# bcsefercik/markerless-robot-camera-calibration

Hardware: AMD Instinct MI355X
Metric: point-cloud frames/sec at 200k pts/frame (higher is better)
Workload: dtype f32

## Files before the change

markerless-robot-camera-calibration_amd/csrc/sv_conv.hip:

```cpp
#include <stdarg.h>
#include <stdio.h>
#include <stdlib.h>
#include <vector>

#include "sv_conv_params.h"

namespace sv {

static thread_local char g_last_instance[128] = "";
static thread_local double g_want_scale_override = -1.0;
static thread_local double g_tail_override = -1.0;
void note_instance(const char* fmt, ...) {
  va_list ap;
  va_start(ap, fmt);
  vsnprintf(g_last_instance, sizeof(g_last_instance), fmt, ap);
  va_end(ap);
}
#ifndef SV_CONV_WANT_SCALE_DEFAULT
#define SV_CONV_WANT_SCALE_DEFAULT 0.3
#endif
#ifndef SV_CONV_TAIL_DEFAULT
#define SV_CONV_TAIL_DEFAULT 0.15
#endif
constexpr int chunk_for(int tm, int waves_n) {
  if (waves_n == 1) return tm <= 64 ? 128 : 64;
  if (waves_n == 2) return tm <= 32 ? 128 : (tm <= 64 ? 64 : 32);
  return tm <= 16 ? 128 : (tm <= 32 ? 64 : 32);
}

constexpr int fused_offsets(int cpo) { return cpo == 0 ? 1 : (cpo < 8 ? 27 : (128 / cpo > 0 ? 128 / cpo : 1)); }
constexpr int lds_row_stride(int kc) {
  for (int sa = kc + 2;; ++sa)
    if (sa % 64 == 34 || (sa % 4 == 0 && (sa / 4) % 2 == 1)) return sa;
}

template <int TM_, int WAVES_N, int NT, int CPO = 0>
struct ConvCfg {
  static constexpr int WAVES_M = 4 / WAVES_N;
  static constexpr int MR = TM_ / WAVES_M / 16;
  static constexpr int TN = WAVES_N * NT * 16;
  static constexpr int GK = fused_offsets(CPO);
  static constexpr int KC = CPO ? (GK * CPO + 3) / 4 * 4 : chunk_for(TM_, WAVES_N);
  static constexpr int SA = lds_row_stride(KC);
  static constexpr int PFD_RAW = MR * NT >= 6 ? 1 : (8 + MR * NT - 1) / (MR * NT);
  static constexpr int PFD = PFD_RAW > KC / 4 ? KC / 4 : PFD_RAW;
  static constexpr bool USE_FULL = (MR * NT == 1) || (TM_ == 32 && WAVES_N == 4 && NT == 3) || (TM_ == 16 && NT == 3);
  static constexpr int F4_PER_ROW = KC / 4;
  static constexpr int ROWS_PER_PASS = 256 / F4_PER_ROW;
  static constexpr int A_F4 = (TM_ + ROWS_PER_PASS - 1) / ROWS_PER_PASS;
  static_assert(MR >= 1, "tile too small for the wave layout");
  static constexpr size_t lds_bytes(int K) { return (size_t)(2 * TM_ * SA + K * TM_) * sizeof(float); }
};

template <int TM_, int WAVES_N, int NT, bool FAST, int CPO = 0, bool RING = false, bool FULL = false>
__device__ __forceinline__ void conv_tile_body(const ConvParams& p, const int bidx, const int tile_base) {
  static_assert(FAST || !FULL, "FULL is a refinement of the FAST form");
  using Cfg = ConvCfg<TM_, WAVES_N, NT, CPO>;
  constexpr int MR = Cfg::MR, TN = Cfg::TN, A_F4 = Cfg::A_F4, KC = Cfg::KC, SA = Cfg::SA, GK = Cfg::GK;
  constexpr int PFD = RING ? Cfg::PFD : 1;
  constexpr int ROWS_PER_PASS = Cfg::ROWS_PER_PASS;
  constexpr int SUBS = TM_ / 16;
  extern __shared__ __attribute__((aligned(16))) float lds[];
  float* As = lds;
  int* idx_s = (int*)(lds + 2 * TM_ * SA);

  const int tid = threadIdx.x;
  const int lane = tid & 63;
  const int wid = __builtin_amdgcn_readfirstlane(tid >> 6);
  const int wm = wid / WAVES_N, wn = wid % WAVES_N;
  unsigned long long trace_t0 = 0, trace_t_loop = 0, trace_t_epi = 0;
  int trace_steps = 0;
  if (p.trace) trace_t0 = wall_clock64();
  const int ny = (p.Cout + TN - 1) / TN;
  constexpr int SUB_PER_PLAN_TILE = PLAN_TILE / TM_;
  const int t_lin = bidx / ny;
  const int t128 = tile_base + t_lin / SUB_PER_PLAN_TILE;
  const int p128 = p.tile_order ? p.tile_order[t128] : ((int)(p.Vpad / PLAN_TILE) - 1 - t128);
  const int tile = p128 * SUB_PER_PLAN_TILE + (t_lin % SUB_PER_PLAN_TILE);
  const int n0 = (bidx % ny) * TN;
  const int64_t row0 = (int64_t)tile * TM_;
  const int li = lane & 15, lq = lane >> 4;
  const int K = p.K, Cin = p.Cin, Cout = p.Cout;
  const int col0 = n0 + wn * NT * 16 + NT * li;
  const bool cols_full = col0 + NT <= Cout;

  f32x4 acc[MR][NT];
#pragma unroll
  for (int s = 0; s < MR; ++s)
#pragma unroll
    for (int n = 0; n < NT; ++n) acc[s][n] = (f32x4){0.f, 0.f, 0.f, 0.f};

  if (p.acc_init) {
    if constexpr (FAST) {
      const __amdgpu_buffer_rsrc_t rsrc_acc = __builtin_amdgcn_make_buffer_rsrc((void*)p.acc_init, 0, (int)p.acc_bytes, 0x00020000);
      int o_acc[MR][4];
      load_perm_rows<MR>(p, row0 + wm * MR * 16, lane >> 4, o_acc);
#pragma unroll
      for (int s = 0; s < MR; ++s)
#pragma unroll
        for (int reg = 0; reg < 4; ++reg) {
          const auto v = buffer_load_floats<NT>(
              rsrc_acc, o_acc[s][reg] >= 0 ? (uint32_t)o_acc[s][reg] * (uint32_t)(p.acc_ld * 4) + (uint32_t)col0 * 4u : BUF_ABSENT, 0u);
#pragma unroll
          for (int n = 0; n < NT; ++n) acc[s][n][reg] = v[n];
        }
    } else {
#pragma unroll
      for (int s = 0; s < MR; ++s)
#pragma unroll
        for (int reg = 0; reg < 4; ++reg) {
          const int64_t r = row0 + wm * MR * 16 + s * 16 + (lane >> 4) * 4 + reg;
          const int64_t o = p.perm ? (int64_t)p.perm[r] : (r < p.V_out ? r : -1);
#pragma unroll
          for (int n = 0; n < NT; ++n) acc[s][n][reg] = (o >= 0 && col0 + n < Cout) ? p.acc_init[o * p.acc_ld + col0 + n] : 0.0f;
        }
    }
  }
  uint32_t dense_mask = (1u << SUBS) - 1u;
  if (p.submask == nullptr) {
    const int64_t rem = p.V_out - row0;
    const int nsub = rem >= TM_ ? SUBS : (int)((rem + 15) / 16);
    dense_mask = (1u << nsub) - 1u;
  }
  if constexpr (FAST) {
    constexpr int STAGE_IT = (32 * TM_ + 255) / 256;
    int n_st[STAGE_IT];
#pragma unroll
    for (int it = 0; it < STAGE_IT; ++it) {
      const int e = tid + 256 * it;
      const int k = e / TM_, r = e % TM_;
      n_st[it] = -1;
      if (e < K * TM_) {
        if (p.nbr_s)
          n_st[it] = p.nbr_s[(int64_t)k * p.Vpad + row0 + r];
        else
          n_st[it] = (row0 + r < p.V_out) ? (int)(row0 + r) : -1;
      }
    }
#pragma unroll
    for (int it = 0; it < STAGE_IT; ++it) {
      const int e = tid + 256 * it;
      if (e < K * TM_) idx_s[e] = (int)(n_st[it] >= 0 ? (uint32_t)n_st[it] * (uint32_t)(p.in_ld * 4) : BUF_ABSENT);
    }
  } else {
    for (int e = tid; e < K * TM_; e += 256) {
      const int k = e / TM_, r = e - k * TM_;
      int n;
      if (p.nbr_s)
        n = p.nbr_s[(int64_t)k * p.Vpad + row0 + r];
      else
        n = (row0 + r < p.V_out) ? (int)(row0 + r) : -1;
      idx_s[e] = n;
    }
  }
  const __amdgpu_buffer_rsrc_t rsrc_in = __builtin_amdgcn_make_buffer_rsrc((void*)p.in, 0, (int)p.in_bytes, 0x00020000);
  const __amdgpu_buffer_rsrc_t rsrc_w = __builtin_amdgcn_make_buffer_rsrc((void*)p.W, 0, (int)p.w_bytes, 0x00020000);

  const int64_t sm_word = row0 / PLAN_TILE;
  const int sm_shift = (int)((row0 % PLAN_TILE) / 16);
  uint32_t my_sm = 0;
  if (lane < K) my_sm = p.submask ? ((p.submask[sm_word * K + lane] >> sm_shift) & ((1u << SUBS) - 1u)) : dense_mask;
  const uint32_t amask = (uint32_t)__ballot(my_sm != 0);
  auto fused_mask = [&](int k0) -> uint32_t {
    uint32_t m = 0;
#pragma unroll
    for (int g = 0; g < GK; ++g) m |= (uint32_t)__builtin_amdgcn_readlane((int)my_sm, min(k0 + g, 31));
    return m;
  };
  int k_n, c_n = 0;
  uint32_t sm_n = 0;
  bool have_n;
  if (CPO) {
    k_n = 0;
    while (k_n < K && (sm_n = fused_mask(k_n)) == 0) k_n += GK;
    have_n = k_n < K;
  } else {
    k_n = amask ? __builtin_ctz(amask) : K;
    sm_n = amask ? (uint32_t)__builtin_amdgcn_readlane((int)my_sm, k_n) : 0u;
    have_n = amask != 0;
  }
  auto advance = [&]() {
    if (CPO) {
      k_n += GK;
      while (k_n < K && (sm_n = fused_mask(k_n)) == 0) k_n += GK;
      have_n = k_n < K;
      return;
    }
    c_n += KC;
    if (c_n >= Cin) {
      c_n = 0;
      const uint32_t rest = amask & ~((2u << k_n) - 1u);
      have_n = rest != 0;
      k_n = have_n ? __builtin_ctz(rest) : K;
      sm_n = (uint32_t)__builtin_amdgcn_readlane((int)my_sm, have_n ? k_n : 0);
    }
  };

  float4 ra[A_F4];
  const int a_cc = (tid % Cfg::F4_PER_ROW) * 4;
  const int a_r = tid / Cfg::F4_PER_ROW;

  const uint32_t col_bytes = (uint32_t)a_cc * 4u;
  const int cin_rem = Cin % KC;
  const uint32_t col_last = (cin_rem == 0 || a_cc < cin_rem) ? col_bytes : 0u - (uint32_t)(Cin - cin_rem) * 4u;
  auto load_a = [&](int k, int c0, uint32_t sm) {
#pragma unroll
    for (int j = 0; j < A_F4; ++j) {
      const int r = a_r + ROWS_PER_PASS * j;
      if (FAST) {
        const int rr = (A_F4 * ROWS_PER_PASS > TM_) ? min(r, TM_ - 1) : r;
        if (CPO) {
          const int kk = k + a_cc / (CPO ? CPO : 1);
          uint32_t off = (uint32_t)idx_s[min(kk, K - 1) * TM_ + rr];
          if (kk >= K) off = BUF_ABSENT;
          const f32x4 v = buffer_load_floats<4>(rsrc_in, off + (uint32_t)(a_cc % (CPO ? CPO : 1)) * 4u, 0u);
          ra[j] = make_float4(v[0], v[1], v[2], v[3]);
        } else {
          const uint32_t off = (uint32_t)idx_s[k * TM_ + rr];
          const uint32_t cb = (!FULL && c0 + KC > Cin) ? col_last : col_bytes;
          const f32x4 v = buffer_load_floats<4>(rsrc_in, off + cb, (uint32_t)c0 * 4u);
          ra[j] = make_float4(v[0], v[1], v[2], v[3]);
        }
        (void)sm;
      } else if (CPO) {
        float e[4] = {0.f, 0.f, 0.f, 0.f};
        if (r < TM_ && ((sm >> (r >> 4)) & 1u)) {
#pragma unroll
          for (int q = 0; q < 4; ++q) {
            const int i = a_cc + q, kk = k + i / (CPO ? CPO : 1), c = i % (CPO ? CPO : 1);
            if (i < GK * CPO && kk < K) {
              const int n = idx_s[kk * TM_ + r];
              if (n >= 0) e[q] = p.in[(int64_t)n * p.in_ld + c];
            }
          }
        }
        ra[j] = make_float4(e[0], e[1], e[2], e[3]);
      } else {
        float4 v = make_float4(0.f, 0.f, 0.f, 0.f);
        if (r < TM_ && ((sm >> (r >> 4)) & 1u)) {
          const int n = idx_s[k * TM_ + r];
          const int c = c0 + a_cc;
          if (n >= 0) {
            const float* src = p.in + (int64_t)n * p.in_ld + c;
            if (p.vec_a) {
              if (c < Cin) v = *(const float4*)src;
            } else {
              if (c + 0 < Cin) v.x = src[0];
              if (c + 1 < Cin) v.y = src[1];
              if (c + 2 < Cin) v.z = src[2];
              if (c + 3 < Cin) v.w = src[3];
            }
          }
        }
        ra[j] = v;
      }
    }
  };
  auto store_a = [&](float* dstbuf, uint32_t sm) {
#pragma unroll
    for (int j = 0; j < A_F4; ++j) {
      const int r = a_r + ROWS_PER_PASS * j;
      if (r < TM_ && (FAST || ((sm >> (r >> 4)) & 1u))) {
        float2* dst = (float2*)(dstbuf + r * SA + a_cc);
        dst[0] = make_float2(ra[j].x, ra[j].y);
        dst[1] = make_float2(ra[j].z, ra[j].w);
      }
    }
  };

  typedef float bvec_t __attribute__((ext_vector_type(NT)));
  typedef float bvec_load_t __attribute__((ext_vector_type(NT), aligned(4)));
  bvec_t b[KC / 4];
  const int b_off = lq * Cout + col0;
  const uint32_t b_off_bytes = (uint32_t)b_off * 4u;
  auto step_weights = [&](int k, int c0) -> const float* { return p.W + ((int64_t)k * Cin + c0) * Cout; };
  auto cols_of = [&](int k, int c0) { return CPO ? min(GK, K - k) * CPO : min(KC, Cin - c0); };
  auto ksteps_of = [&](int k, int c0) { return (cols_of(k, c0) + 3) >> 2; };
  auto load_b = [&](const float* wstep, int k, int c0, int ksteps_valid, int ks, bvec_t& dst) {
    if (FAST) {
      const uint32_t row = (uint32_t)(k * Cin + c0 + (ks < ksteps_valid ? 4 * ks : 0));
      dst = buffer_load_floats<NT>(rsrc_w, b_off_bytes, row * (uint32_t)Cout * 4u);
      (void)wstep;
    } else {
      const int i = 4 * ks + lq;
      const float* src = p.W + ((int64_t)k * Cin + c0 + i) * Cout + col0;
      const bool row_ok = i < cols_of(k, c0);
#pragma unroll
      for (int n = 0; n < NT; ++n) dst[n] = (row_ok && col0 + n < Cout) ? src[n] : 0.0f;
    }
  };

  __syncthreads();
  if (have_n) {
    int k_c = k_n, c_c = c_n;
    uint32_t sm_c = sm_n;
    load_a(k_c, c_c, sm_c);
#pragma unroll
    for (int ks = 0; ks < KC / 4; ++ks) load_b(step_weights(k_c, c_c), k_c, c_c, ksteps_of(k_c, c_c), ks, b[ks]);
    store_a(As, sm_c);
    advance();
    int k_x = k_n, c_x = c_n;
    uint32_t sm_x = sm_n;
    bool have_x = have_n;
    __syncthreads();
    int buf = 0;
    if (p.trace) trace_t_loop = wall_clock64();

    auto step = [&]() -> bool {
      if (FAST || have_x) load_a(have_x ? k_x : 0, have_x ? c_x : 0, have_x ? sm_x : 0u);
      const float* a_base = As + buf * (TM_ * SA) + (wm * MR * 16 + li) * SA + lq;
      const uint32_t smw = (sm_c >> (wm * MR)) & ((1u << MR) - 1u);
      const int ksteps = ksteps_of(k_c, c_c);
      const int kb = have_x ? k_x : 0;
      const int cb = have_x ? c_x : 0;
      const float* wnext = step_weights(kb, cb);
      const int ksteps_next = ksteps_of(kb, cb);
      {
        auto reload_b = [&](int ks) {
          if (FULL) {
            b[ks] = buffer_load_floats<NT>(rsrc_w, b_off_bytes, (uint32_t)(kb * Cin + cb + 4 * ks) * (uint32_t)Cout * 4u);
          } else if (FAST || have_x) {
            load_b(wnext, kb, cb, ksteps_next, ks, b[ks]);
          }
        };
        auto mfma_row = [&](int ks, const float (&a)[MR]) {
#pragma unroll
          for (int s = 0; s < MR; ++s) {
            if ((MR == 1 && Cfg::WAVES_M == 1) || ((smw >> s) & 1u)) {
#pragma unroll
              for (int n = 0; n < NT; ++n)
                acc[s][n] = __builtin_amdgcn_mfma_f32_16x16x4f32(a[s], b[ks][n], acc[s][n], 0, 0, 0);
            }
          }
        };
        if constexpr (PFD == 1) {
          float a_cur[MR];
#pragma unroll
          for (int s = 0; s < MR; ++s) a_cur[s] = a_base[s * 16 * SA];
#pragma unroll
          for (int ks = 0; ks < KC / 4; ++ks) {
            if (FULL || ks < ksteps) {
              float a_nx[MR];
              if (ks + 1 < KC / 4) {
#pragma unroll
                for (int s = 0; s < MR; ++s) a_nx[s] = a_base[s * 16 * SA + (ks + 1) * 4];
                if (FULL) __builtin_amdgcn_sched_barrier(0);
              }
              mfma_row(ks, a_cur);
              if (ks + 1 < KC / 4) {
#pragma unroll
                for (int s = 0; s < MR; ++s) a_cur[s] = a_nx[s];
              }
            }
            reload_b(ks);
            if (FULL) __builtin_amdgcn_sched_barrier(0);
          }
        } else {
          float a_ring[PFD + 1][MR];
#pragma unroll
          for (int d = 0; d < PFD; ++d)
#pragma unroll
            for (int s = 0; s < MR; ++s) a_ring[d][s] = a_base[s * 16 * SA + d * 4];
#pragma unroll
          for (int ks = 0; ks < KC / 4; ++ks) {
            if (FULL || ks < ksteps) {
              if (ks + PFD < KC / 4) {
#pragma unroll
                for (int s = 0; s < MR; ++s)
                  a_ring[(ks + PFD) % (PFD + 1)][s] = a_base[s * 16 * SA + (ks + PFD) * 4];
                if (FULL) __builtin_amdgcn_sched_barrier(0);
              }
              mfma_row(ks, a_ring[ks % (PFD + 1)]);
            }
            reload_b(ks);
            if (FULL) __builtin_amdgcn_sched_barrier(0);
          }
        }
      }
      ++trace_steps;
      if (!have_x) return false;
      store_a(As + (buf ^ 1) * (TM_ * SA), sm_x);
      k_c = k_x;
      c_c = c_x;
      sm_c = sm_x;
      advance();
      k_x = k_n;
      c_x = c_n;
      sm_x = sm_n;
      have_x = have_n;
      __syncthreads();
      buf ^= 1;
      return true;
    };
    while (step()) {
    }
  }

  if (p.trace) trace_t_epi = wall_clock64();
  float sc[NT], sh[NT];
#pragma unroll
  for (int n = 0; n < NT; ++n) {
    const bool ok = col0 + n < Cout;
    sc[n] = (p.scale && ok) ? p.scale[col0 + n] : 1.0f;
    sh[n] = (p.shift && ok) ? p.shift[col0 + n] : 0.0f;
  }
  if constexpr (FAST) {
    epilogue_buffered<MR, NT>(p, acc, row0 + wm * MR * 16, lq, col0);
  } else
#pragma unroll
  for (int s = 0; s < MR; ++s) {
#pragma unroll
    for (int reg = 0; reg < 4; ++reg) {
      const int64_t r = row0 + wm * MR * 16 + s * 16 + lq * 4 + reg;
      int64_t o;
      if (p.perm)
        o = p.perm[r];
      else
        o = (r < p.V_out) ? r : -1;
      if (o < 0) continue;
      float y[NT];
#pragma unroll
      for (int n = 0; n < NT; ++n) {
        float v = acc[s][n][reg];
        if (p.scale)
          v = __builtin_fmaf(v, sc[n], sh[n]);
        else if (p.shift)
          v = v + sh[n];
        y[n] = v;
      }
      if (p.residual) {
        const float* res = p.residual + o * p.res_ld + col0;
#pragma unroll
        for (int n = 0; n < NT; ++n)
          if (col0 + n < Cout) y[n] = y[n] + res[n];
      }
      float* dst = p.out + o * p.out_ld + col0;
#pragma unroll
      for (int n = 0; n < NT; ++n) {
        float v = y[n];
        if (p.act == SV_ACT_RELU)
          v = v < 0.f ? 0.f : v;
        else if (p.act == SV_ACT_LEAKY_RELU)
          v = v > 0.f ? v : v * p.slope;
        if (col0 + n < Cout) dst[n] = v;
      }
    }
  }
  if (p.trace && tid == 0) {
    unsigned long long* t = p.trace + (size_t)blockIdx.x * 4;
    t[0] = trace_t0;
    t[1] = wall_clock64();
    t[2] = ((unsigned long long)__builtin_amdgcn_s_getreg((31 << 11) | 20) << 32) |
           (unsigned)__builtin_amdgcn_s_getreg((31 << 11) | 4);
    const unsigned long long pro = trace_t_loop ? ((trace_t_loop - trace_t0) >> 4) & 0xffffull : 0ull;
    const unsigned long long epi = ((t[1] - trace_t_epi) >> 4) & 0xffffull;
    t[3] = (unsigned long long)(unsigned)trace_steps | (pro << 32) | (epi << 48);
  }
}

template <int TM_, int WAVES_N, int NT, bool FAST, int CPO = 0, bool RING = false, bool FULL = false>
__global__ __launch_bounds__(256) void conv_fwd_kernel(ConvParams p) {
  conv_tile_body<TM_, WAVES_N, NT, FAST, CPO, RING, FULL>(p, (int)blockIdx.x, 0);
}

template <int TM_, int TAIL_TM, int WAVES_N, int NT, bool FAST>
__global__ __launch_bounds__(256) void conv_fwd_dual_kernel(ConvParams p) {
  if ((int)blockIdx.x < p.main_blocks)
    conv_tile_body<TM_, WAVES_N, NT, FAST>(p, (int)blockIdx.x, 0);
  else
    conv_tile_body<TAIL_TM, WAVES_N, NT, FAST>(p, (int)blockIdx.x - p.main_blocks, p.main_tiles128);
}

template <class Launch>
static int launch_traced(ConvParams& q, unsigned grid, int tm, int wn, int nt, hipStream_t stream, Launch&& launch) {
  static const char* trace_path = getenv("SV_CONV_TRACE");
  q.trace = nullptr;
  if (trace_path) SV_HIP(hipMalloc((void**)&q.trace, (size_t)grid * 4 * sizeof(unsigned long long)));
  launch();
  SV_LAUNCH_CHECK();
  if (q.trace) {
    std::vector<unsigned long long> host((size_t)grid * 4);
    SV_HIP(hipStreamSynchronize(stream));
    SV_HIP(hipMemcpy(host.data(), q.trace, host.size() * sizeof(unsigned long long), hipMemcpyDeviceToHost));
    SV_HIP(hipFree(q.trace));
    if (FILE* f = fopen(trace_path, "ab")) {
      const long long hdr[8] = {0x5356545243ll, (long long)grid, tm, wn, nt, q.ny, q.K, q.Cin};
      fwrite(hdr, sizeof(hdr), 1, f);
      fwrite(host.data(), sizeof(unsigned long long), host.size(), f);
      fclose(f);
    }
  }
  return SV_OK;
}

template <int TM_, int WAVES_N, int NT, int CPO = 0>
static int launch_conv(const ConvParams& p, hipStream_t stream) {
  using Cfg = ConvCfg<TM_, WAVES_N, NT, CPO>;
  ConvParams q = p;
  q.ntiles = (int)(p.Vpad / TM_);
  q.ny = (p.Cout + Cfg::TN - 1) / Cfg::TN;
  dim3 grid((unsigned)(q.ntiles * q.ny));
  const bool fast = p.vec_a && p.buf_ok && (p.Cout % Cfg::TN == 0);
  const bool ring = Cfg::PFD > 1 && grid.x <= 1024;
  constexpr bool F = (CPO % 4 == 0);
  const size_t lds = Cfg::lds_bytes(p.K);
  const bool full = Cfg::USE_FULL && (CPO ? (p.K % Cfg::GK == 0) : (p.Cin % Cfg::KC == 0));
  const int rc = launch_traced(q, grid.x, TM_, WAVES_N, NT, stream, [&] {
    if (F && fast && full) {
      if (ring)
        hipLaunchKernelGGL((conv_fwd_kernel<TM_, WAVES_N, NT, F, CPO, (Cfg::PFD > 1), (F && Cfg::USE_FULL)>), grid, dim3(256), lds, stream, q);
      else
        hipLaunchKernelGGL((conv_fwd_kernel<TM_, WAVES_N, NT, F, CPO, false, (F && Cfg::USE_FULL)>), grid, dim3(256), lds, stream, q);
    } else if (F && fast) {
      if (ring)
        hipLaunchKernelGGL((conv_fwd_kernel<TM_, WAVES_N, NT, F, CPO, (Cfg::PFD > 1)>), grid, dim3(256), lds, stream, q);
      else
        hipLaunchKernelGGL((conv_fwd_kernel<TM_, WAVES_N, NT, F, CPO, false>), grid, dim3(256), lds, stream, q);
    } else {
      if (ring)
        hipLaunchKernelGGL((conv_fwd_kernel<TM_, WAVES_N, NT, false, CPO, (Cfg::PFD > 1)>), grid, dim3(256), lds, stream, q);
      else
        hipLaunchKernelGGL((conv_fwd_kernel<TM_, WAVES_N, NT, false, CPO, false>), grid, dim3(256), lds, stream, q);
    }
  });
  if (rc != SV_OK) return rc;
  {
    const bool f = F && fast;
    if (CPO)
      note_instance("conv_fwd_kernel<%d, %d, %d, fused %d>|fast=%d,ring=%d,full=%d", TM_, WAVES_N, NT, CPO, (int)f, (int)ring,
                    (int)(f && full));
    else
      note_instance("conv_fwd_kernel<%d, %d, %d>|fast=%d,ring=%d,full=%d", TM_, WAVES_N, NT, (int)f, (int)ring, (int)(f && full));
  }
  return SV_OK;
}

template <int TM_, int TAIL_TM, int WAVES_N, int NT>
static int launch_conv_dual(const ConvParams& p, hipStream_t stream, double tail_fraction) {
  using Main = ConvCfg<TM_, WAVES_N, NT, 0>;
  using Tail = ConvCfg<TAIL_TM, WAVES_N, NT, 0>;
  const bool fast = p.vec_a && p.buf_ok && (p.Cout % Main::TN == 0);
  const int n128 = (int)(p.Vpad / PLAN_TILE);
  const int tail128 = (int)(n128 * tail_fraction);
  if (!fast || !p.tile_order || tail128 < 1 || tail128 >= n128) return SV_ERR_INVALID;
  ConvParams q = p;
  q.ny = p.Cout / Main::TN;
  q.main_tiles128 = n128 - tail128;
  q.main_blocks = q.main_tiles128 * (PLAN_TILE / TM_) * q.ny;
  q.ntiles = (int)(p.Vpad / TM_);
  const unsigned grid = (unsigned)(q.main_blocks + tail128 * (PLAN_TILE / TAIL_TM) * q.ny);
  const size_t lds = Main::lds_bytes(p.K) > Tail::lds_bytes(p.K) ? Main::lds_bytes(p.K) : Tail::lds_bytes(p.K);
  const int rc = launch_traced(q, grid, TM_, WAVES_N, NT, stream, [&] {
    hipLaunchKernelGGL((conv_fwd_dual_kernel<TM_, TAIL_TM, WAVES_N, NT, true>), dim3(grid), dim3(256), lds, stream, q);
  });
  if (rc != SV_OK) return rc;
  note_instance("conv_fwd_dual_kernel<%d, %d, %d, %d>|fast=1,ring=0,full=0", TM_, TAIL_TM, WAVES_N, NT);
  return SV_OK;
}

struct Candidate {
  int tm, wn, nt;
  int64_t want;
  int cpo;
};

template <int TM_, int WAVES_N, int NT, int CPO = 0>
static bool try_launch(const Candidate& c, const ConvParams& p, hipStream_t stream, int& rc) {
  if (c.tm == TM_ && c.wn == WAVES_N && c.nt == NT && c.cpo == CPO) {
    rc = launch_conv<TM_, WAVES_N, NT, CPO>(p, stream);
    return true;
  }
  return false;
}

static int launch_candidate(const Candidate& c, const ConvParams& p, hipStream_t stream) {
  int rc = SV_ERR_INVALID;
  if (try_launch<128, 4, 3>(c, p, stream, rc) || try_launch<128, 2, 3>(c, p, stream, rc) ||
      try_launch<128, 1, 3>(c, p, stream, rc) || try_launch<64, 4, 3>(c, p, stream, rc) ||
      try_launch<64, 2, 3>(c, p, stream, rc) || try_launch<64, 1, 3>(c, p, stream, rc) ||
      try_launch<32, 4, 3>(c, p, stream, rc) || try_launch<32, 2, 3>(c, p, stream, rc) ||
      try_launch<16, 4, 3>(c, p, stream, rc) ||
      try_launch<128, 4, 2>(c, p, stream, rc) || try_launch<128, 2, 2>(c, p, stream, rc) ||
      try_launch<128, 1, 2>(c, p, stream, rc) || try_launch<64, 4, 2>(c, p, stream, rc) ||
      try_launch<64, 2, 2>(c, p, stream, rc) || try_launch<64, 1, 2>(c, p, stream, rc) ||
      try_launch<32, 4, 2>(c, p, stream, rc) || try_launch<32, 2, 2>(c, p, stream, rc) ||
      try_launch<16, 4, 2>(c, p, stream, rc) ||
      try_launch<64, 4, 1>(c, p, stream, rc) || try_launch<32, 4, 1>(c, p, stream, rc) ||
      try_launch<16, 4, 1>(c, p, stream, rc) || try_launch<128, 2, 1>(c, p, stream, rc) ||
      try_launch<64, 2, 1>(c, p, stream, rc) || try_launch<32, 2, 1>(c, p, stream, rc) ||
      try_launch<128, 1, 1>(c, p, stream, rc) || try_launch<64, 1, 1>(c, p, stream, rc) ||
      try_launch<64, 2, 1, 3>(c, p, stream, rc) || try_launch<32, 2, 1, 3>(c, p, stream, rc) ||
      try_launch<64, 2, 1, 32>(c, p, stream, rc) || try_launch<32, 2, 1, 32>(c, p, stream, rc) ||
      try_launch<32, 4, 1, 32>(c, p, stream, rc) || try_launch<16, 4, 1, 32>(c, p, stream, rc) ||
      try_launch<32, 4, 1, 64>(c, p, stream, rc) || try_launch<16, 4, 1, 64>(c, p, stream, rc))
    return rc;
  set_error("sv_conv_fwd: no kernel instance <%d,%d,%d> cpo %d", c.tm, c.wn, c.nt, c.cpo);
  return SV_ERR_INVALID;
}

static int64_t candidate_wgs(const Candidate& c, const ConvParams& p) {
  const int tn = c.wn * c.nt * 16;
  return (p.Vpad / c.tm) * ((p.Cout + tn - 1) / tn);
}

static int select_and_launch(const ConvParams& p, hipStream_t stream) {
  static const Candidate wide3[] = {{64, 4, 3, 2500}, {32, 4, 3, 1500}, {32, 2, 3, 0}};
  static const Candidate wide3_128[] = {{64, 4, 3, 2500}, {64, 4, 2, 1200}, {32, 4, 3, 1200}, {16, 4, 3, 0}};
  static const Candidate wide3_128_full[] = {{64, 4, 3, 2500}, {32, 4, 3, 1200}, {16, 4, 3, 0}};
  static const Candidate wide2[] = {{128, 4, 2, 1300}, {64, 4, 2, 1500}, {32, 4, 2, 1500}, {32, 2, 2, 0}};
  static const Candidate wide2_64[] = {{128, 4, 2, 1300}, {64, 4, 2, 1500}, {32, 4, 2, 1500}, {16, 4, 1, 0}};
  static const Candidate c64[] = {{64, 4, 1, 1500}, {32, 4, 1, 1500}, {16, 4, 1, 0}};
  static const Candidate c32[] = {{128, 2, 1, 1500}, {64, 2, 1, 1500}, {32, 2, 1, 0}};
  static const Candidate c16[] = {{128, 1, 1, 600}, {64, 1, 1, 0}};
  const Candidate* list;
  int n;
  const int Cout = p.Cout;
  if (Cout > 128 && (Cout % 192 == 0 || Cout % 96 == 0 || Cout > 2048)) {
    if (Cout % 128 != 0) { list = wide3; n = 3; }
    else if (p.Cin % 128 == 0 && p.vec_a) { list = wide3_128_full; n = 3; }
    else { list = wide3_128; n = 4; }
  }
  else if (Cout > 64) { list = Cout % 64 == 0 ? wide2_64 : wide2; n = 4; }
  else if (Cout > 32) { list = c64; n = 3; }
  else if (Cout > 16) { list = c32; n = 3; }
  else { list = c16; n = 2; }
  static const Candidate f3[] = {{64, 2, 1, 3000, 3}, {32, 2, 1, 0, 3}};
  static const Candidate f32_32[] = {{64, 2, 1, 3000, 32}, {32, 2, 1, 0, 32}};
  static const Candidate f32_64[] = {{32, 4, 1, 1500, 32}, {16, 4, 1, 0, 32}};
  static const Candidate f64_64[] = {{32, 4, 1, 1500, 64}, {16, 4, 1, 0, 64}};
  if (p.K > 1) {
    if (p.Cin == 3 && Cout > 16 && Cout <= 32) { list = f3; n = 2; }
    else if (p.Cin == 32 && p.vec_a && Cout == 32) { list = f32_32; n = 2; }
    else if (p.Cin == 32 && p.vec_a && Cout == 64) { list = f32_64; n = 2; }
    else if (p.Cin == 64 && p.vec_a && (Cout == 64 || Cout == 128)) { list = f64_64; n = 2; }
  }
  if (const char* f = getenv("SV_CONV_FORCE_RANGE")) {
    long long vmin = 0, vmax = 0;
    int cout = 0;
    Candidate c = {0, 0, 0, 0, 0};
    if (sscanf(f, "%lld:%lld:%d:%d,%d,%d", &vmin, &vmax, &cout, &c.tm, &c.wn, &c.nt) == 6 && p.Vpad >= vmin && p.Vpad <= vmax &&
        p.Cout == cout && p.K > 1)
      return launch_candidate(c, p, stream);
  }
  if (const char* f = getenv("SV_CONV_FORCE_DENSE")) {
    long long vmin = 0;
    int cout = 0;
    Candidate c = {0, 0, 0, 0, 0};
    if (sscanf(f, "%lld:%d:%d,%d,%d", &vmin, &cout, &c.tm, &c.wn, &c.nt) == 5 && p.Vpad >= vmin && p.Cout == cout && p.K == 1)
      return launch_candidate(c, p, stream);
  }
  if (const char* f = getenv("SV_CONV_FORCE")) {
    Candidate c = {0, 0, 0, 0, 0};
    if (sscanf(f, "%d,%d,%d,%d", &c.tm, &c.wn, &c.nt, &c.cpo) >= 3) return launch_candidate(c, p, stream);
  }
  static const double want_scale =
      getenv("SV_CONV_WANT_SCALE") ? atof(getenv("SV_CONV_WANT_SCALE")) : SV_CONV_WANT_SCALE_DEFAULT;
  static const double tail_fraction = getenv("SV_CONV_TAIL") ? atof(getenv("SV_CONV_TAIL")) : SV_CONV_TAIL_DEFAULT;
  const double ws = g_want_scale_override >= 0.0 ? g_want_scale_override : want_scale;
  const double tf = g_tail_override >= 0.0 ? g_tail_override : tail_fraction;
  for (int i = 0; i < n; ++i)
    if ((double)candidate_wgs(list[i], p) >= ws * (double)list[i].want) {
      const Candidate& c = list[i];
      if (c.tm == 64 && c.wn == 4 && c.nt == 3 && c.cpo == 0 && tf > 0.0 &&
          launch_conv_dual<64, 32, 4, 3>(p, stream, tf) == SV_OK)
        return SV_OK;
      return launch_candidate(c, p, stream);
    }
  return launch_candidate(list[n - 1], p, stream);
}

}

using namespace sv;

extern "C" const char* sv_conv_last_instance(void) { return sv::g_last_instance; }

extern "C" int sv_conv_set_dispatch(double want_scale, double tail_fraction) {
  SV_CHECK_ARG(tail_fraction < 1.0, "tail_fraction must be below 1");
  sv::g_want_scale_override = want_scale;
  sv::g_tail_override = tail_fraction;
  return SV_OK;
}

extern "C" int sv_conv_fwd(const float* in, int64_t V_in, int64_t in_ld, int Cin, const float* W, int K, int Cout,
                           const int32_t* perm, const int32_t* nbr_s, const uint32_t* submask,
                           const int32_t* tile_order, int64_t V_out, int64_t Vpad, const float* scale, const float* shift, const float* residual, int64_t res_ld,
                           int act, float slope, float* out, int64_t out_ld, sv_stream_t stream_) {
  return sv_conv_fwd_acc(in, V_in, in_ld, Cin, W, K, Cout, perm, nbr_s, submask, tile_order, V_out, Vpad, nullptr, 0, scale, shift,
                         residual, res_ld, act, slope, out, out_ld, stream_);
}

extern "C" int sv_conv_fwd_acc(const float* in, int64_t V_in, int64_t in_ld, int Cin, const float* W, int K, int Cout,
                               const int32_t* perm, const int32_t* nbr_s, const uint32_t* submask, const int32_t* tile_order,
                               int64_t V_out, int64_t Vpad, const float* acc_init, int64_t acc_ld, const float* scale,
                               const float* shift, const float* residual, int64_t res_ld, int act, float slope, float* out,
                               int64_t out_ld, sv_stream_t stream_) {
  hipStream_t stream = (hipStream_t)stream_;
  SV_CHECK_ARG(!acc_init || acc_ld >= Cout, "acc_init stride too small");
  SV_CHECK_ARG(Cin > 0 && Cout > 0 && K >= 1 && K <= 32, "bad channel / kernel volume");
  SV_CHECK_ARG(V_out >= 0 && Vpad >= V_out && Vpad % PLAN_TILE == 0, "Vpad must be a multiple of 128 >= V_out");
  SV_CHECK_ARG(in_ld >= Cin && out_ld >= Cout, "row strides too small");
  SV_CHECK_ARG(act >= SV_ACT_NONE && act <= SV_ACT_LEAKY_RELU, "bad activation");
  if (V_out == 0) return SV_OK;
  SV_CHECK_ARG(in && W && out, "null pointer");
  SV_CHECK_ARG(V_in >= 1, "V_in = rows of `in` (every index of the plan is below it)");
  const bool has_plan = perm || nbr_s || submask;
  SV_CHECK_ARG(!has_plan || (perm && nbr_s && submask), "perm, nbr_s and submask must be given together");
  SV_CHECK_ARG(has_plan || K == 1, "K > 1 needs a plan");
  SV_CHECK_ARG(!residual || res_ld >= Cout, "residual stride too small");
  ConvParams p;
  p.in = in; p.in_ld = in_ld; p.Cin = Cin; p.W = W; p.K = K; p.Cout = Cout;
  p.perm = perm; p.nbr_s = nbr_s; p.submask = submask; p.tile_order = tile_order; p.V_out = V_out; p.Vpad = Vpad;
  p.scale = scale; p.shift = shift; p.residual = residual; p.res_ld = res_ld;
  p.acc_init = acc_init; p.acc_ld = acc_ld;
  p.act = act; p.slope = slope; p.out = out; p.out_ld = out_ld;
  p.vec_a = (in_ld % 4 == 0) && (Cin % 4 == 0) && (((uintptr_t)in & 15) == 0);
  const uint64_t in_bytes = ((uint64_t)(V_in - 1) * (uint64_t)in_ld + (uint64_t)Cin) * 4u;
  const uint64_t w_bytes = (uint64_t)K * (uint64_t)Cin * (uint64_t)Cout * 4u;
  const uint64_t out_bytes = ((uint64_t)(V_out - 1) * (uint64_t)out_ld + (uint64_t)Cout) * 4u;
  const uint64_t res_bytes = residual ? ((uint64_t)(V_out - 1) * (uint64_t)res_ld + (uint64_t)Cout) * 4u : 0u;
  const uint64_t acc_bytes = acc_init ? ((uint64_t)(V_out - 1) * (uint64_t)acc_ld + (uint64_t)Cout) * 4u : 0u;
  p.buf_ok = in_bytes < BUF_LIMIT && w_bytes < BUF_LIMIT && out_bytes < BUF_LIMIT && res_bytes < BUF_LIMIT &&
             acc_bytes < BUF_LIMIT && (((uintptr_t)perm & 15) == 0);
  p.acc_bytes = p.buf_ok ? (uint32_t)acc_bytes : 0u;
  if (!p.buf_ok && !has_plan && K == 1 && w_bytes < BUF_LIMIT) {
    int64_t ld_max = in_ld > out_ld ? in_ld : out_ld;
    if (residual && res_ld > ld_max) ld_max = res_ld;
    const int64_t rows = (int64_t)((BUF_LIMIT - 4096u) / ((uint64_t)ld_max * 4u)) / PLAN_TILE * PLAN_TILE;
    if (rows >= PLAN_TILE && rows < V_out) {
      for (int64_t r0 = 0; r0 < V_out; r0 += rows) {
        const int64_t n = V_out - r0 < rows ? V_out - r0 : rows;
        const int rc = sv_conv_fwd_acc(in + r0 * in_ld, n, in_ld, Cin, W, K, Cout, nullptr, nullptr, nullptr, nullptr, n,
                                       (n + PLAN_TILE - 1) / PLAN_TILE * PLAN_TILE, acc_init ? acc_init + r0 * acc_ld : nullptr,
                                       acc_ld, scale, shift, residual ? residual + r0 * res_ld : nullptr, res_ld, act, slope,
                                       out + r0 * out_ld, out_ld, stream_);
        if (rc != SV_OK) return rc;
      }
      return SV_OK;
    }
  }
  p.in_bytes = p.buf_ok ? (uint32_t)in_bytes : 0u;
  p.w_bytes = p.buf_ok ? (uint32_t)w_bytes : 0u;
  p.out_bytes = p.buf_ok ? (uint32_t)out_bytes : 0u;
  p.res_bytes = p.buf_ok ? (uint32_t)res_bytes : 0u;
  p.ntiles = 0;
  p.ny = 0;
  p.trace = nullptr;
  p.main_blocks = 0;
  p.main_tiles128 = 0;
  if (has_plan && K > 1 && K <= 27 && Cin == 3 && Cout == 32 && !acc_init) {
    if (p.buf_ok) return launch_conv_first_mfma(p, stream);
    return launch_conv_first_layer(p, stream);
  }
  if (has_plan && K > 1 && K <= 32 && Cin == 32 && Cout == 32 && p.vec_a && p.buf_ok && !acc_init)
    return launch_conv_thin(p, stream, sv::g_want_scale_override >= 1.0);
  if (!has_plan && K == 1 && Cout <= 4 && p.vec_a && Cin >= 64 && !acc_init) return launch_linear_narrow(p, stream);
  return select_and_launch(p, stream);
}
```

markerless-robot-camera-calibration_amd/csrc/sv_conv_params.h:

```cpp
#pragma once
#include <type_traits>

#include "sv_common.h"

namespace sv {

typedef float f32x4 __attribute__((ext_vector_type(4)));

struct ConvParams {
  const float* in;
  int64_t in_ld;
  int Cin;
  const float* W;
  int K;
  int Cout;
  const int32_t* perm;
  const int32_t* nbr_s;
  const uint32_t* submask;
  const int32_t* tile_order;
  int64_t V_out;
  int64_t Vpad;
  const float* scale;
  const float* shift;
  const float* residual;
  int64_t res_ld;
  const float* acc_init;
  int64_t acc_ld;
  uint32_t acc_bytes;
  int act;
  float slope;
  float* out;
  int64_t out_ld;
  int vec_a;
  uint32_t in_bytes, w_bytes, out_bytes, res_bytes;
  int buf_ok;
  int ntiles;
  int ny;
  unsigned long long* trace;
  int main_blocks;
  int main_tiles128;
};

constexpr int PLAN_TILE = SV_TILE_ROWS;
void note_instance(const char* fmt, ...);
int launch_conv_first_mfma(const ConvParams& p, hipStream_t stream);
int launch_conv_first_layer(const ConvParams& p, hipStream_t stream);
int launch_conv_thin(const ConvParams& p, hipStream_t stream, bool alone);
int launch_linear_narrow(const ConvParams& p, hipStream_t stream);

constexpr uint32_t BUF_ABSENT = 0x80000000u;
constexpr uint32_t BUF_LIMIT = 0x7fff0000u;
typedef int i32x4_t __attribute__((ext_vector_type(4)));
typedef int i32x3_t __attribute__((ext_vector_type(3)));
typedef int i32x2_t __attribute__((ext_vector_type(2)));
template <int N>
__device__ __forceinline__ auto buffer_load_floats(__amdgpu_buffer_rsrc_t rsrc, uint32_t voffset, uint32_t soffset) {
  typedef float vec_t __attribute__((ext_vector_type(N)));
  if constexpr (N == 1) {
    vec_t r;
    r[0] = __builtin_bit_cast(float, __builtin_amdgcn_raw_buffer_load_b32(rsrc, voffset, soffset, 0));
    return r;
  } else if constexpr (N == 2) {
    return __builtin_bit_cast(vec_t, __builtin_amdgcn_raw_buffer_load_b64(rsrc, voffset, soffset, 0));
  } else if constexpr (N == 3) {
    return __builtin_bit_cast(vec_t, __builtin_amdgcn_raw_buffer_load_b96(rsrc, voffset, soffset, 0));
  } else {
    static_assert(N == 4, "1..4 floats per load");
    return __builtin_bit_cast(vec_t, __builtin_amdgcn_raw_buffer_load_b128(rsrc, voffset, soffset, 0));
  }
}

template <int MR>
__device__ __forceinline__ void load_perm_rows(const ConvParams& p, const int64_t rows0, const int lq, int (&o)[MR][4]) {
#pragma unroll
  for (int s = 0; s < MR; ++s) {
    const int64_t r = rows0 + s * 16 + lq * 4;
    if (p.perm) {
      const int4 o4 = *(const int4*)(p.perm + r);
      o[s][0] = o4.x;
      o[s][1] = o4.y;
      o[s][2] = o4.z;
      o[s][3] = o4.w;
    } else {
#pragma unroll
      for (int reg = 0; reg < 4; ++reg) o[s][reg] = (r + reg < p.V_out) ? (int)(r + reg) : -1;
    }
  }
}

template <int MR, int NT, bool PRELOADED = false>
__device__ __forceinline__ void epilogue_buffered(const ConvParams& p, const f32x4 (&acc)[MR][NT], const int64_t rows0,
                                                  const int lq, const int col0, const int (*o_pre)[4] = nullptr) {
  typedef float yvec_t __attribute__((ext_vector_type(NT)));
  const __amdgpu_buffer_rsrc_t rsrc_out = __builtin_amdgcn_make_buffer_rsrc((void*)p.out, 0, (int)p.out_bytes, 0x00020000);
  const __amdgpu_buffer_rsrc_t rsrc_res =
      __builtin_amdgcn_make_buffer_rsrc((void*)p.residual, 0, p.residual ? (int)p.res_bytes : 0, 0x00020000);
  int o[MR][4];
  if constexpr (PRELOADED) {
#pragma unroll
    for (int s = 0; s < MR; ++s)
#pragma unroll
      for (int reg = 0; reg < 4; ++reg) o[s][reg] = o_pre[s][reg];
  } else {
    load_perm_rows<MR>(p, rows0, lq, o);
  }
  float scf[NT], shf[NT];
#pragma unroll
  for (int n = 0; n < NT; ++n) {
    scf[n] = p.scale ? p.scale[col0 + n] : 1.0f;
    shf[n] = p.shift ? p.shift[col0 + n] : (p.scale ? 0.0f : -0.0f);
  }
  const float slope = p.slope;
  auto finish = [&](auto act_tag) {
    constexpr int ACT = decltype(act_tag)::value;
#pragma unroll
    for (int s = 0; s < MR; ++s) {
      yvec_t res[4];
#pragma unroll
      for (int reg = 0; reg < 4; ++reg)
#pragma unroll
        for (int n = 0; n < NT; ++n) res[reg][n] = -0.0f;
      if (p.residual) {
#pragma unroll
        for (int reg = 0; reg < 4; ++reg)
          res[reg] = buffer_load_floats<NT>(
              rsrc_res, o[s][reg] >= 0 ? (uint32_t)o[s][reg] * (uint32_t)(p.res_ld * 4) + (uint32_t)col0 * 4u : BUF_ABSENT,
              0u);
      }
#pragma unroll
      for (int reg = 0; reg < 4; ++reg) {
        yvec_t y;
#pragma unroll
        for (int n = 0; n < NT; ++n) {
          float v = __builtin_fmaf(acc[s][n][reg], scf[n], shf[n]) + res[reg][n];
          if constexpr (ACT == SV_ACT_RELU)
            v = v < 0.f ? 0.f : v;
          else if constexpr (ACT == SV_ACT_LEAKY_RELU)
            v = v > 0.f ? v : v * slope;
          y[n] = v;
        }
        const uint32_t off =
            o[s][reg] >= 0 ? (uint32_t)o[s][reg] * (uint32_t)(p.out_ld * 4) + (uint32_t)col0 * 4u : BUF_ABSENT;
        if constexpr (NT == 1)
          __builtin_amdgcn_raw_buffer_store_b32(__builtin_bit_cast(int, y[0]), rsrc_out, off, 0, 0);
        else if constexpr (NT == 2)
          __builtin_amdgcn_raw_buffer_store_b64(__builtin_bit_cast(i32x2_t, y), rsrc_out, off, 0, 0);
        else if constexpr (NT == 3)
          __builtin_amdgcn_raw_buffer_store_b96(__builtin_bit_cast(i32x3_t, y), rsrc_out, off, 0, 0);
        else
          __builtin_amdgcn_raw_buffer_store_b128(__builtin_bit_cast(i32x4_t, y), rsrc_out, off, 0, 0);
      }
    }
  };
  if (p.act == SV_ACT_RELU)
    finish(std::integral_constant<int, SV_ACT_RELU>{});
  else if (p.act == SV_ACT_LEAKY_RELU)
    finish(std::integral_constant<int, SV_ACT_LEAKY_RELU>{});
  else
    finish(std::integral_constant<int, SV_ACT_NONE>{});
}

}
```

Measured before the change: 73.83.

## Add dense 1x1 conv path and stage output permutation in LDS

Adds a DENSE template variant for K==1 convolutions without a neighbor map. It computes input row offsets directly and skips the idx_s staging, the submask handling and the initial barrier. In the sparse fast path, the output permutation is staged into LDS once and reused by the acc_init load and the epilogue. The first A-tile load is issued before the acc_init loads so their latencies overlap. The cost is more LDS per block and extra kernel instantiations.

Result: no change. 74.06, median of 6 (+0.3%).

```diff
diff --git a/markerless-robot-camera-calibration_amd/csrc/sv_conv.hip b/markerless-robot-camera-calibration_amd/csrc/sv_conv.hip
--- a/markerless-robot-camera-calibration_amd/csrc/sv_conv.hip
+++ b/markerless-robot-camera-calibration_amd/csrc/sv_conv.hip
@@ -49,12 +49,13 @@
   static constexpr int ROWS_PER_PASS = 256 / F4_PER_ROW;
   static constexpr int A_F4 = (TM_ + ROWS_PER_PASS - 1) / ROWS_PER_PASS;
   static_assert(MR >= 1, "tile too small for the wave layout");
-  static constexpr size_t lds_bytes(int K) { return (size_t)(2 * TM_ * SA + K * TM_) * sizeof(float); }
+  static constexpr size_t lds_bytes(int K) { return (size_t)(2 * TM_ * SA + K * TM_ + TM_) * sizeof(float); }
 };
 
-template <int TM_, int WAVES_N, int NT, bool FAST, int CPO = 0, bool RING = false, bool FULL = false>
+template <int TM_, int WAVES_N, int NT, bool FAST, int CPO = 0, bool RING = false, bool FULL = false, bool DENSE = false>
 __device__ __forceinline__ void conv_tile_body(const ConvParams& p, const int bidx, const int tile_base) {
   static_assert(FAST || !FULL, "FULL is a refinement of the FAST form");
+  static_assert(!DENSE || (FAST && CPO == 0), "DENSE is a refinement of the FAST one-offset-per-step form");
   using Cfg = ConvCfg<TM_, WAVES_N, NT, CPO>;
   constexpr int MR = Cfg::MR, TN = Cfg::TN, A_F4 = Cfg::A_F4, KC = Cfg::KC, SA = Cfg::SA, GK = Cfg::GK;
   constexpr int PFD = RING ? Cfg::PFD : 1;
@@ -63,6 +64,7 @@
   extern __shared__ __attribute__((aligned(16))) float lds[];
   float* As = lds;
   int* idx_s = (int*)(lds + 2 * TM_ * SA);
+  int* perm_s = idx_s + p.K * TM_;
 
   const int tid = threadIdx.x;
   const int lane = tid & 63;
@@ -90,21 +92,8 @@
 #pragma unroll
     for (int n = 0; n < NT; ++n) acc[s][n] = (f32x4){0.f, 0.f, 0.f, 0.f};
 
-  if (p.acc_init) {
-    if constexpr (FAST) {
-      const __amdgpu_buffer_rsrc_t rsrc_acc = __builtin_amdgcn_make_buffer_rsrc((void*)p.acc_init, 0, (int)p.acc_bytes, 0x00020000);
-      int o_acc[MR][4];
-      load_perm_rows<MR>(p, row0 + wm * MR * 16, lane >> 4, o_acc);
-#pragma unroll
-      for (int s = 0; s < MR; ++s)
-#pragma unroll
-        for (int reg = 0; reg < 4; ++reg) {
-          const auto v = buffer_load_floats<NT>(
-              rsrc_acc, o_acc[s][reg] >= 0 ? (uint32_t)o_acc[s][reg] * (uint32_t)(p.acc_ld * 4) + (uint32_t)col0 * 4u : BUF_ABSENT, 0u);
-#pragma unroll
-          for (int n = 0; n < NT; ++n) acc[s][n][reg] = v[n];
-        }
-    } else {
+  if constexpr (!FAST) {
+    if (p.acc_init) {
 #pragma unroll
       for (int s = 0; s < MR; ++s)
 #pragma unroll
@@ -119,12 +108,19 @@
   uint32_t dense_mask = (1u << SUBS) - 1u;
   if (p.submask == nullptr) {
     const int64_t rem = p.V_out - row0;
-    const int nsub = rem >= TM_ ? SUBS : (int)((rem + 15) / 16);
+    const int nsub = rem >= TM_ ? SUBS : (rem > 0 ? (int)((rem + 15) / 16) : 0);
     dense_mask = (1u << nsub) - 1u;
   }
-  if constexpr (FAST) {
-    constexpr int STAGE_IT = (32 * TM_ + 255) / 256;
-    int n_st[STAGE_IT];
+  const int64_t sm_word = row0 / PLAN_TILE;
+  const int sm_shift = (int)((row0 % PLAN_TILE) / 16);
+  uint32_t my_sm = 0;
+  if constexpr (!DENSE) {
+    if (lane < K) my_sm = p.submask ? ((p.submask[sm_word * K + lane] >> sm_shift) & ((1u << SUBS) - 1u)) : dense_mask;
+  }
+  constexpr int STAGE_IT = (32 * TM_ + 255) / 256;
+  int n_st[STAGE_IT];
+  int o_st = -1;
+  if constexpr (FAST && !DENSE) {
 #pragma unroll
     for (int it = 0; it < STAGE_IT; ++it) {
       const int e = tid + 256 * it;
@@ -137,12 +133,8 @@
           n_st[it] = (row0 + r < p.V_out) ? (int)(row0 + r) : -1;
       }
     }
-#pragma unroll
-    for (int it = 0; it < STAGE_IT; ++it) {
-      const int e = tid + 256 * it;
-      if (e < K * TM_) idx_s[e] = (int)(n_st[it] >= 0 ? (uint32_t)n_st[it] * (uint32_t)(p.in_ld * 4) : BUF_ABSENT);
-    }
-  } else {
+    if (tid < TM_) o_st = p.perm ? p.perm[row0 + tid] : ((row0 + tid < p.V_out) ? (int)(row0 + tid) : -1);
+  } else if constexpr (!FAST) {
     for (int e = tid; e < K * TM_; e += 256) {
       const int k = e / TM_, r = e - k * TM_;
       int n;
@@ -156,11 +148,7 @@
   const __amdgpu_buffer_rsrc_t rsrc_in = __builtin_amdgcn_make_buffer_rsrc((void*)p.in, 0, (int)p.in_bytes, 0x00020000);
   const __amdgpu_buffer_rsrc_t rsrc_w = __builtin_amdgcn_make_buffer_rsrc((void*)p.W, 0, (int)p.w_bytes, 0x00020000);
 
-  const int64_t sm_word = row0 / PLAN_TILE;
-  const int sm_shift = (int)((row0 % PLAN_TILE) / 16);
-  uint32_t my_sm = 0;
-  if (lane < K) my_sm = p.submask ? ((p.submask[sm_word * K + lane] >> sm_shift) & ((1u << SUBS) - 1u)) : dense_mask;
-  const uint32_t amask = (uint32_t)__ballot(my_sm != 0);
+  const uint32_t amask = DENSE ? (dense_mask != 0) : (uint32_t)__ballot(my_sm != 0);
   auto fused_mask = [&](int k0) -> uint32_t {
     uint32_t m = 0;
 #pragma unroll
@@ -170,7 +158,11 @@
   int k_n, c_n = 0;
   uint32_t sm_n = 0;
   bool have_n;
-  if (CPO) {
+  if (DENSE) {
+    k_n = 0;
+    sm_n = dense_mask;
+    have_n = dense_mask != 0;
+  } else if (CPO) {
     k_n = 0;
     while (k_n < K && (sm_n = fused_mask(k_n)) == 0) k_n += GK;
     have_n = k_n < K;
@@ -180,6 +172,11 @@
     have_n = amask != 0;
   }
   auto advance = [&]() {
+    if (DENSE) {
+      c_n += KC;
+      have_n = c_n < Cin;
+      return;
+    }
     if (CPO) {
       k_n += GK;
       while (k_n < K && (sm_n = fused_mask(k_n)) == 0) k_n += GK;
@@ -203,6 +200,8 @@
   const uint32_t col_bytes = (uint32_t)a_cc * 4u;
   const int cin_rem = Cin % KC;
   const uint32_t col_last = (cin_rem == 0 || a_cc < cin_rem) ? col_bytes : 0u - (uint32_t)(Cin - cin_rem) * 4u;
+  const uint32_t a_off0 = DENSE ? (uint32_t)(row0 + a_r) * (uint32_t)(p.in_ld * 4) : 0u;
+  const uint32_t a_pass_bytes = (uint32_t)ROWS_PER_PASS * (uint32_t)(p.in_ld * 4);
   auto load_a = [&](int k, int c0, uint32_t sm) {
 #pragma unroll
     for (int j = 0; j < A_F4; ++j) {
@@ -216,9 +215,9 @@
           const f32x4 v = buffer_load_floats<4>(rsrc_in, off + (uint32_t)(a_cc % (CPO ? CPO : 1)) * 4u, 0u);
           ra[j] = make_float4(v[0], v[1], v[2], v[3]);
         } else {
-          const uint32_t off = (uint32_t)idx_s[k * TM_ + rr];
+          const uint32_t off = DENSE ? a_off0 : (uint32_t)idx_s[k * TM_ + rr];
           const uint32_t cb = (!FULL && c0 + KC > Cin) ? col_last : col_bytes;
-          const f32x4 v = buffer_load_floats<4>(rsrc_in, off + cb, (uint32_t)c0 * 4u);
+          const f32x4 v = buffer_load_floats<4>(rsrc_in, off + cb, (uint32_t)c0 * 4u + (DENSE ? (uint32_t)j * a_pass_bytes : 0u));
           ra[j] = make_float4(v[0], v[1], v[2], v[3]);
         }
         (void)sm;
@@ -290,11 +289,38 @@
     }
   };
 
-  __syncthreads();
+  if constexpr (FAST && !DENSE) {
+#pragma unroll
+    for (int it = 0; it < STAGE_IT; ++it) {
+      const int e = tid + 256 * it;
+      if (e < K * TM_) idx_s[e] = (int)(n_st[it] >= 0 ? (uint32_t)n_st[it] * (uint32_t)(p.in_ld * 4) : BUF_ABSENT);
+    }
+    if (tid < TM_) perm_s[tid] = o_st;
+  }
+  if constexpr (!DENSE) __syncthreads();
+  if (have_n) load_a(k_n, c_n, sm_n);
+  if constexpr (FAST) {
+    if (p.acc_init) {
+      const __amdgpu_buffer_rsrc_t rsrc_acc = __builtin_amdgcn_make_buffer_rsrc((void*)p.acc_init, 0, (int)p.acc_bytes, 0x00020000);
+      int o_acc[MR][4];
+      if constexpr (DENSE)
+        load_perm_rows<MR>(p, row0 + wm * MR * 16, lq, o_acc);
+      else
+        load_perm_rows_lds<MR>(perm_s + wm * MR * 16, lq, o_acc);
+#pragma unroll
+      for (int s = 0; s < MR; ++s)
+#pragma unroll
+        for (int reg = 0; reg < 4; ++reg) {
+          const auto v = buffer_load_floats<NT>(
+              rsrc_acc, o_acc[s][reg] >= 0 ? (uint32_t)o_acc[s][reg] * (uint32_t)(p.acc_ld * 4) + (uint32_t)col0 * 4u : BUF_ABSENT, 0u);
+#pragma unroll
+          for (int n = 0; n < NT; ++n) acc[s][n][reg] = v[n];
+        }
+    }
+  }
   if (have_n) {
     int k_c = k_n, c_c = c_n;
     uint32_t sm_c = sm_n;
-    load_a(k_c, c_c, sm_c);
 #pragma unroll
     for (int ks = 0; ks < KC / 4; ++ks) load_b(step_weights(k_c, c_c), k_c, c_c, ksteps_of(k_c, c_c), ks, b[ks]);
     store_a(As, sm_c);
@@ -405,7 +431,13 @@
     sh[n] = (p.shift && ok) ? p.shift[col0 + n] : 0.0f;
   }
   if constexpr (FAST) {
-    epilogue_buffered<MR, NT>(p, acc, row0 + wm * MR * 16, lq, col0);
+    if constexpr (DENSE) {
+      epilogue_buffered<MR, NT>(p, acc, row0 + wm * MR * 16, lq, col0);
+    } else {
+      int o_epi[MR][4];
+      load_perm_rows_lds<MR>(perm_s + wm * MR * 16, lq, o_epi);
+      epilogue_buffered<MR, NT, true>(p, acc, row0 + wm * MR * 16, lq, col0, o_epi);
+    }
   } else
 #pragma unroll
   for (int s = 0; s < MR; ++s) {
@@ -458,9 +490,9 @@
   }
 }
 
-template <int TM_, int WAVES_N, int NT, bool FAST, int CPO = 0, bool RING = false, bool FULL = false>
+template <int TM_, int WAVES_N, int NT, bool FAST, int CPO = 0, bool RING = false, bool FULL = false, bool DENSE = false>
 __global__ __launch_bounds__(256) void conv_fwd_kernel(ConvParams p) {
-  conv_tile_body<TM_, WAVES_N, NT, FAST, CPO, RING, FULL>(p, (int)blockIdx.x, 0);
+  conv_tile_body<TM_, WAVES_N, NT, FAST, CPO, RING, FULL, DENSE>(p, (int)blockIdx.x, 0);
 }
 
 template <int TM_, int TAIL_TM, int WAVES_N, int NT, bool FAST>
@@ -505,8 +537,20 @@
   constexpr bool F = (CPO % 4 == 0);
   const size_t lds = Cfg::lds_bytes(p.K);
   const bool full = Cfg::USE_FULL && (CPO ? (p.K % Cfg::GK == 0) : (p.Cin % Cfg::KC == 0));
+  constexpr bool D = F && CPO == 0;
+  const bool dense = D && fast && !p.nbr_s && p.K == 1;
   const int rc = launch_traced(q, grid.x, TM_, WAVES_N, NT, stream, [&] {
-    if (F && fast && full) {
+    if (dense && full) {
+      if (ring)
+        hipLaunchKernelGGL((conv_fwd_kernel<TM_, WAVES_N, NT, F, CPO, (Cfg::PFD > 1), (F && Cfg::USE_FULL), D>), grid, dim3(256), lds, stream, q);
+      else
+        hipLaunchKernelGGL((conv_fwd_kernel<TM_, WAVES_N, NT, F, CPO, false, (F && Cfg::USE_FULL), D>), grid, dim3(256), lds, stream, q);
+    } else if (dense) {
+      if (ring)
+        hipLaunchKernelGGL((conv_fwd_kernel<TM_, WAVES_N, NT, F, CPO, (Cfg::PFD > 1), false, D>), grid, dim3(256), lds, stream, q);
+      else
+        hipLaunchKernelGGL((conv_fwd_kernel<TM_, WAVES_N, NT, F, CPO, false, false, D>), grid, dim3(256), lds, stream, q);
+    } else if (F && fast && full) {
       if (ring)
         hipLaunchKernelGGL((conv_fwd_kernel<TM_, WAVES_N, NT, F, CPO, (Cfg::PFD > 1), (F && Cfg::USE_FULL)>), grid, dim3(256), lds, stream, q);
       else
diff --git a/markerless-robot-camera-calibration_amd/csrc/sv_conv_params.h b/markerless-robot-camera-calibration_amd/csrc/sv_conv_params.h
--- a/markerless-robot-camera-calibration_amd/csrc/sv_conv_params.h
+++ b/markerless-robot-camera-calibration_amd/csrc/sv_conv_params.h
@@ -88,6 +88,18 @@
   }
 }
 
+template <int MR>
+__device__ __forceinline__ void load_perm_rows_lds(const int* perm_rows, const int lq, int (&o)[MR][4]) {
+#pragma unroll
+  for (int s = 0; s < MR; ++s) {
+    const int4 o4 = *(const int4*)(perm_rows + s * 16 + lq * 4);
+    o[s][0] = o4.x;
+    o[s][1] = o4.y;
+    o[s][2] = o4.z;
+    o[s][3] = o4.w;
+  }
+}
+
 template <int MR, int NT, bool PRELOADED = false>
 __device__ __forceinline__ void epilogue_buffered(const ConvParams& p, const f32x4 (&acc)[MR][NT], const int64_t rows0,
                                                   const int lq, const int col0, const int (*o_pre)[4] = nullptr) {
```
